# samanseifi/pyRMT

Hardware: AMD Instinct MI355X
Metric: cell-updates/s (full RMT step) at N=4096; achieved HBM GB/s vs peak (higher is better)
Workload: dtype f64; 1 GPU; soft_disc_in_lid_driven N=4096 semilagrangian (configs 2/4 loop body); grid=4096, parallelism=single-gpu

## Files before the change

include/rmt.h:

```cpp
#ifndef RMT_H
#define RMT_H

#ifdef __cplusplus
extern "C" {
#endif

typedef enum {
    RMT_OK = 0,
    RMT_EINVAL = 1,
    RMT_ENONFINITE = 2,
    RMT_EDEVICE = 3,
    RMT_ENOTSUP = 4,
    RMT_ENOMEM = 5
} rmt_status;

typedef enum {
    RMT_BC_NONE = 0,
    RMT_BC_NOSLIP_LID = 1,
    RMT_BC_FREESLIP_BOX = 2,
    RMT_BC_PERIODIC = 3
} rmt_bc_kind;

typedef enum {
    RMT_SCHEME_SEMILAGRANGIAN = 0,
// ... 54 lines not shown
int rmt_extrap_last_path(rmt_ctx *ctx, int *path);

int rmt_rebuild_phi_disc(rmt_ctx *ctx, const double *X1, const double *X2, double x0, double y0,
                         double R, double *phi);

int rmt_solid_cauchy_stress(rmt_ctx *ctx, const double *X1, const double *X2, double dx,
                            double dy, double mu_s, double kappa, const double *phi,
                            double w_cut, double detg_clamp, int isochoric, double *sxx,
                            double *sxy, double *syy, double *J);
int rmt_smoothed_heaviside(rmt_ctx *ctx, const double *x, long n, double w_t, double *H);
int rmt_apply_velocity_bc(rmt_ctx *ctx, int bc_kind, double lid, double *u, double *v);

typedef struct {
    int bc_kind;
    double lid;
    double mu_s, kappa, eta_s, rho_s, rho_f, mu_f, w_t;
    double dx, dy, dt;
    int stress_band;
    double detg_clamp;
} rmt_momentum_params;

int rmt_momentum_step_rk4(rmt_ctx *ctx, const rmt_momentum_params *prm, const double *u,
                          const double *v, const double *p, const double *X1, const double *X2,
                          const double *phi, double *u_new, double *v_new, double *sxx,
                          double *sxy, double *syy, double *J);
int rmt_compute_curvature(rmt_ctx *ctx, const double *phi, double dx, double dy, double *kappa);
int rmt_compute_contact_force(rmt_ctx *ctx, const double *phi1, const double *phi2, double k_rep,
                              double w_c, double dx, double dy, double *fx, double *fy);
int rmt_momentum_step_rk4_st(rmt_ctx *ctx, const rmt_momentum_params *prm, double gamma,
                             const double *u, const double *v, const double *p, const double *X1,
                             const double *X2, const double *phi, double *u_new, double *v_new,
                             double *sxx, double *sxy, double *syy, double *J);
int rmt_momentum_step_rk4_2solids(rmt_ctx *ctx, const rmt_momentum_params *prm, double k_rep,
                                  double w_c, const double *u, const double *v, const double *p,
                                  const double *X1a, const double *X2a, const double *X1b,
                                  const double *X2b, const double *phi_a, const double *phi_b,
                                  double *u_new, double *v_new, double *Jmin);

int rmt_mask_solid(rmt_ctx *ctx, const double *q, const double *phi, double *out);
int rmt_mixture_density(rmt_ctx *ctx, const double *phi_a, const double *phi_b, double w_t,
                        double rho_s, double rho_f, double *rho);
int rmt_two_solid_diag(rmt_ctx *ctx, const double *phi_a, const double *phi_b, const double *X,
                       const double *Y, const double *Jmin, double *out5);

int rmt_momentum_set_mode(int mode);

int rmt_divergence_rc(rmt_ctx *ctx, const double *a, const double *b, const double *p,
                      double d_f, double dx, double dy, double *divU);
int rmt_divergence_central(rmt_ctx *ctx, const double *a, const double *b, double dx,
                           double dy, double *divU);
int rmt_pressure_gradient(rmt_ctx *ctx, const double *p, double dx, double dy, double *gx,
                          double *gy);
int rmt_solve_poisson_dct(rmt_ctx *ctx, const double *rhs, double dx, double dy, double *p);
int rmt_pressure_projection(rmt_ctx *ctx, const double *a_star, const double *b_star,
                            double dx, double dy, double dt, double rho, int bc_kind,
                            double lid, const double *p_prev, double *a, double *b, double *p);
int rmt_pressure_projection_rho_field(rmt_ctx *ctx, const double *a_star, const double *b_star,
                                      double dx, double dy, double dt, const double *rho,
                                      int bc_kind, double lid, const double *p_prev, double *a,
                                      double *b, double *p);
int rmt_pressure_projection_variable(rmt_ctx *ctx, const double *a_star, const double *b_star,
                                     double dx, double dy, double dt, const double *rho,
                                     int bc_kind, double lid, const double *p_prev, double rtol,
                                     int maxiter, double *a, double *b, double *p, int *iters);
int rmt_apply_variable_poisson(rmt_ctx *ctx, const double *p, double dx, double dy,
                               const double *inv_rho, double *out);
int rmt_divergence_rc_variable(rmt_ctx *ctx, const double *a, const double *b, const double *p,
                               double dt, const double *rho, double dx, double dy,
                               double *divU);

int rmt_compute_timestep(rmt_ctx *ctx, const double *a, const double *b, double dx, double dy,
                         double CFL, double dt_min_cap, double mu_s, double rho_s, double gamma,
                         double rho_f, double mu_f, double eta_s, double kappa, double *dt);

int rmt_compute_kinetic_energy(rmt_ctx *ctx, const double *a, const double *b, double rho_f,
                               double rho_s, const double *phi, double w_t, double dx, double dy,
                               double *ke);
int rmt_compute_strain_energy(rmt_ctx *ctx, const double *X1, const double *X2, const double *phi,
                              double mu_s, double dx, double dy, double kappa, double *se);
int rmt_compute_viscous_dissipation(rmt_ctx *ctx, const double *a, const double *b, double mu_f,
                                    const double *phi, double w_t, double dx, double dy,
                                    double eta_s, double *diss);
int rmt_divergence_2d_interior(rmt_ctx *ctx, const double *u, const double *v, double dx,
                               double dy, int pad, double *div);
int rmt_velocity_rhs_blended(rmt_ctx *ctx, const double *u, const double *v, const double *p,
                             const double *sxx, const double *sxy, const double *syy, double dx,
                             double dy, double mu_f, const double *H, const double *rho,
                             const double *fx, const double *fy, double *rhs_u, double *rhs_v);

typedef enum {
    RMT_SHAPE_NONE = 0,
    RMT_SHAPE_DISC = 1
} rmt_shape_kind;

typedef struct {
    int ny, nx;
    double dx, dy;
    const double *xs, *ys;
    int scheme;
    int bc_kind;
    double lid;
    int shape;
    double x0, y0, R;
    double mu_s, kappa, rho_s, eta_s, mu_f, rho_f, w_t;
    int layers;
    double cfl, dt_cap;
// ... 142 lines not shown
```

pyrmt_amd/_lib.py:

```python
import ctypes
import os

_HERE = os.path.dirname(os.path.abspath(__file__))
LIB_PATH = os.environ.get("RMT_LIB") or os.path.join(_HERE, "librmt.so")

RMT_OK, RMT_EINVAL, RMT_ENONFINITE, RMT_EDEVICE, RMT_ENOTSUP, RMT_ENOMEM = range(6)


class RMTError(RuntimeError):
    pass


class rmt_momentum_params(ctypes.Structure):
    _fields_ = [("bc_kind", ctypes.c_int), ("lid", ctypes.c_double),
                ("mu_s", ctypes.c_double), ("kappa", ctypes.c_double),
                ("eta_s", ctypes.c_double), ("rho_s", ctypes.c_double),
                ("rho_f", ctypes.c_double), ("mu_f", ctypes.c_double), ("w_t", ctypes.c_double),
                ("dx", ctypes.c_double), ("dy", ctypes.c_double), ("dt", ctypes.c_double),
                ("stress_band", ctypes.c_int), ("detg_clamp", ctypes.c_double)]


class rmt_sim_params(ctypes.Structure):
    _fields_ = [("ny", ctypes.c_int), ("nx", ctypes.c_int),
                ("dx", ctypes.c_double), ("dy", ctypes.c_double),
# ... 30 lines not shown


_P, _D, _I, _L = ctypes.c_void_p, ctypes.c_double, ctypes.c_int, ctypes.c_long
SIGNATURES = {
    "rmt_last_error": (ctypes.c_char_p, []),
    "rmt_version": (_I, []),
    "rmt_ctx_create": (_I, [_I, _I, _I, _P, ctypes.POINTER(_P)]),
    "rmt_ctx_set_stream": (_I, [_P, _P]),
    "rmt_ctx_destroy": (_I, [_P]),
    "rmt_ctx_sync": (_I, [_P]),
    "rmt_ctx_set_profiling": (_I, [_P, _I]),
    "rmt_ctx_kernel_ms": (_I, [_P, ctypes.POINTER(_D)]),
    "rmt_ctx_set_option": (_I, [_P, ctypes.c_char_p, _I]),
    "rmt_ctx_get_option": (_I, [_P, ctypes.c_char_p, ctypes.POINTER(_I)]),
    "rmt_grad_x_2nd": (_I, [_P, _P, _D, _P]),
    "rmt_grad_y_2nd": (_I, [_P, _P, _D, _P]),
    "rmt_diff_upwind_3rd": (_I, [_P, _P, _P, _D, _I, _P]),
    "rmt_bilinear_interpolate": (_I, [_P, _P, _P, _P, _L, _D, _D, _P]),
    "rmt_advect_sl_rk4": (_I, [_P, _P, _P, _P, _P, _P, _D, _D, _D, _P]),
    "rmt_weno5_rhs": (_I, [_P, _P, _P, _P, _D, _D, _P, _D, _P]),
    "rmt_advect_weno5_rk3": (_I, [_P, _P, _P, _P, _D, _D, _D, _P, _D, _P]),
    "rmt_all_finite2": (_I, [_P, _P, _P, ctypes.POINTER(_I)]),
    "rmt_selftest_divk": (_I, [_P, _P, _L, _D, _P, _P]),
    "rmt_central_rhs": (_I, [_P, _P, _P, _P, _D, _D, _P, _D, _I, _P]),
    "rmt_advect_central_rk3": (_I, [_P, _P, _P, _P, _D, _D, _D, _P, _D, _I, _P]),
    "rmt_bicubic_interpolate": (_I, [_P, _P, _P, _P, _L, _D, _D, _P]),
    "rmt_advect_sl_cubic_rk4": (_I, [_P, _P, _P, _P, _P, _P, _D, _D, _D, _P]),
    "rmt_extrapolate_reference_map": (_I, [_P, _P, _P, _P, _D, _D, _I, _P, _P]),
    "rmt_extrap_set_mode": (_I, [_I]),
    "rmt_extrap_set_parallel": (_I, [_I]),
    "rmt_momentum_set_mode": (_I, [_I]),
    "rmt_extrap_last_path": (_I, [_P, ctypes.POINTER(_I)]),
    "rmt_rebuild_phi_disc": (_I, [_P, _P, _P, _D, _D, _D, _P]),
    "rmt_solid_cauchy_stress": (_I, [_P, _P, _P, _D, _D, _D, _D, _P, _D, _D, _I, _P, _P, _P, _P]),
    "rmt_smoothed_heaviside": (_I, [_P, _P, _L, _D, _P]),
    "rmt_apply_velocity_bc": (_I, [_P, _I, _D, _P, _P]),
    "rmt_momentum_step_rk4": (_I, [_P, ctypes.POINTER(rmt_momentum_params), _P, _P, _P, _P, _P,
                                   _P, _P, _P, _P, _P, _P, _P]),
    "rmt_compute_curvature": (_I, [_P, _P, _D, _D, _P]),
    "rmt_compute_contact_force": (_I, [_P, _P, _P, _D, _D, _D, _D, _P, _P]),
    "rmt_momentum_step_rk4_st": (_I, [_P, ctypes.POINTER(rmt_momentum_params), _D, _P, _P, _P,
                                      _P, _P, _P, _P, _P, _P, _P, _P, _P]),
    "rmt_momentum_step_rk4_2solids": (_I, [_P, ctypes.POINTER(rmt_momentum_params), _D, _D, _P,
                                           _P, _P, _P, _P, _P, _P, _P, _P, _P, _P, _P]),
    "rmt_mask_solid": (_I, [_P, _P, _P, _P]),
    "rmt_mixture_density": (_I, [_P, _P, _P, _D, _D, _D, _P]),
    "rmt_two_solid_diag": (_I, [_P, _P, _P, _P, _P, _P, ctypes.POINTER(_D)]),
    "rmt_pressure_projection_rho_field": (_I, [_P, _P, _P, _D, _D, _D, _P, _I, _D, _P, _P, _P,
                                               _P]),
    "rmt_divergence_rc": (_I, [_P, _P, _P, _P, _D, _D, _D, _P]),
    "rmt_divergence_central": (_I, [_P, _P, _P, _D, _D, _P]),
    "rmt_pressure_gradient": (_I, [_P, _P, _D, _D, _P, _P]),
    "rmt_solve_poisson_dct": (_I, [_P, _P, _D, _D, _P]),
    "rmt_pressure_projection": (_I, [_P, _P, _P, _D, _D, _D, _D, _I, _D, _P, _P, _P, _P]),
    "rmt_pressure_projection_variable": (_I, [_P, _P, _P, _D, _D, _D, _P, _I, _D, _P, _D, _I,
                                              _P, _P, _P, ctypes.POINTER(_I)]),
    "rmt_apply_variable_poisson": (_I, [_P, _P, _D, _D, _P, _P]),
    "rmt_divergence_rc_variable": (_I, [_P, _P, _P, _P, _D, _P, _D, _D, _P]),
    "rmt_compute_timestep": (_I, [_P, _P, _P, _D, _D, _D, _D, _D, _D, _D, _D, _D, _D, _D,
                                  ctypes.POINTER(_D)]),
    "rmt_divergence_2d_interior": (_I, [_P, _P, _P, _D, _D, _I, _P]),
    "rmt_compute_kinetic_energy": (_I, [_P, _P, _P, _D, _D, _P, _D, _D, _D, ctypes.POINTER(_D)]),
    "rmt_compute_strain_energy": (_I, [_P, _P, _P, _P, _D, _D, _D, _D, ctypes.POINTER(_D)]),
    "rmt_compute_viscous_dissipation": (_I, [_P, _P, _P, _D, _P, _D, _D, _D, _D,
                                             ctypes.POINTER(_D)]),
    "rmt_velocity_rhs_blended": (_I, [_P, _P, _P, _P, _P, _P, _P, _D, _D, _D, _P, _P, _P, _P,
                                      _P, _P]),
    "rmt_sim_create": (_I, [_P, ctypes.POINTER(rmt_sim_params), ctypes.POINTER(_P)]),
    "rmt_sim_destroy": (_I, [_P]),
    "rmt_sim_set_sync_every": (_I, [_P, _I]),
    "rmt_sim_field": (_I, [_P, _I, ctypes.POINTER(_P)]),
    "rmt_sim_step": (_I, [_P, _I, _D]),
    "rmt_sim_diagnostics": (_I, [_P, ctypes.POINTER(rmt_diag), _I, ctypes.POINTER(_I)]),
    "rmt_sim_set_profiling": (_I, [_P, _I]),
    "rmt_sim_set_carry": (_I, [_P, _I]),
    "rmt_sim_invalidate": (_I, [_P]),
    "rmt_sim_phase_times": (_I, [_P, ctypes.POINTER(_D), ctypes.POINTER(_L)]),
    "rmt_divergence_periodic": (_I, [_P, _P, _P, _D, _D, _P]),
    "rmt_pressure_gradient_periodic": (_I, [_P, _P, _D, _D, _P, _P]),
    "rmt_solve_poisson_fft": (_I, [_P, _P, _P, _P, _P]),
    "rmt_pressure_projection_periodic": (_I, [_P, _P, _P, _D, _D, _D, _D, _P, _I, _D, _P, _P,
                                              _P, _P, _P, _P]),
    "rmt_slab_create": (_I, [_P, ctypes.POINTER(rmt_sim_params), _I, _I, ctypes.POINTER(_I),
                             ctypes.POINTER(_I), ctypes.POINTER(_P)]),
    "rmt_slab_destroy": (_I, [_P]),
    "rmt_slab_info": (_I, [_P, ctypes.POINTER(_I), ctypes.POINTER(_D)]),
    "rmt_slab_buffer": (_I, [_P, _I, ctypes.POINTER(_P)]),
    "rmt_slab_begin": (_I, [_P]),
    "rmt_slab_advect_interior": (_I, [_P, _D]),
    "rmt_slab_advect": (_I, [_P, _D]),
    "rmt_slab_rim_pack": (_I, [_P]),
    "rmt_slab_extrapolate": (_I, [_P, _P, ctypes.POINTER(ctypes.c_longlong), ctypes.c_longlong]),
    "rmt_slab_momentum": (_I, [_P, _D]),
    "rmt_slab_project_rows": (_I, [_P, _D]),
    "rmt_slab_project_cols": (_I, [_P]),
    "rmt_slab_project_unrows": (_I, [_P]),
    "rmt_slab_sub_mean": (_I, [_P, _I, _P]),
    "rmt_slab_project_correct": (_I, [_P, _D]),
    "rmt_slab_finish": (_I, [_P]),
    "rmt_slab_set_device_dt": (_I, [_P, _I]),
    "rmt_slab_next_dt": (_I, [_P, _P, _I, _P]),
    "rmt_slab_rim_cap": (_I, [_P, ctypes.c_longlong]),
    "rmt_slab_next_bits": (_I, [_P]),
    "rmt_slab_geometry": (_I, [_P]),
    "rmt_slab_drop_geometry": (_I, [_P]),
    "rmt_slab_extrapolate_dev": (_I, [_P, _P, _P, ctypes.c_longlong]),
# ... 72 lines not shown
```

pyrmt_amd/csrc/ops.hip:

```cpp
#include "rmt_internal.hpp"
#include <algorithm>
#include <cstdio>
#include <cstring>
#include <mutex>
#include <vector>

namespace rmt {
static thread_local std::string g_err;
void set_error(const std::string &m) { g_err = m; }
static const struct { const char *name, *env; int rmt_opts::*f; } kOpts[] = {
    {"ext_events", "RMT_EXT_EVENTS", &rmt_opts::ext_events},
    {"ex_arena_bump", nullptr, &rmt_opts::ex_arena_bump},
    {"ex_profile", "RMT_EX_PROFILE", &rmt_opts::ex_profile},
    {"fix_all", "RMT_FIX_ALL", &rmt_opts::fix_all},
    {"dct_rocfft", "RMT_DCT_ROCFFT", &rmt_opts::dct_rocfft},
    {"transpose2", "RMT_TRANSPOSE2", &rmt_opts::transpose2},
    {"sim_hiprio", "RMT_SIM_HIPRIO", &rmt_opts::sim_hiprio},
    {"sim_sync", "RMT_SIM_SYNC", &rmt_opts::sim_sync},
    {"early_geometry", "RMT_EARLY_GEOMETRY", &rmt_opts::early_geometry},
    {"early_transpose", "RMT_EARLY_TRANSPOSE", &rmt_opts::early_transpose},
    {"fused_fluid", "RMT_FUSED_FLUID", &rmt_opts::fused_fluid},
    {"no_overlap", "RMT_NO_OVERLAP", &rmt_opts::no_overlap},
    {"side_tail", "RMT_SIDE_TAIL", &rmt_opts::side_tail},
    {"par_overlap", "RMT_PAR_OVERLAP", &rmt_opts::par_overlap},
    {"fused_fixprep", "RMT_FUSED_FIXPREP", &rmt_opts::fused_fixprep},
    {"merged_join", "RMT_MERGED_JOIN", &rmt_opts::merged_join},
    {"test_delay_side", "RMT_TEST_DELAY_SIDE", &rmt_opts::test_delay_side},
    {"test_delay_main", "RMT_TEST_DELAY_MAIN", &rmt_opts::test_delay_main},
    {"test_delay_geo", "RMT_TEST_DELAY_GEO", &rmt_opts::test_delay_geo},
    {"test_nowait_drop", "RMT_TEST_NOWAIT_DROP", &rmt_opts::test_nowait_drop},
    {"chain_cols", "RMT_CH_PARTS", &rmt_opts::ch_cols},
    {"chain_layer_groups", "RMT_CH_LAYERS", &rmt_opts::ch_lgroups},
    {"edge_slots", "RMT_EDGE_SLOTS_USED", &rmt_opts::edge_slots},
    {"edge_stream", "RMT_EDGE_STREAM", &rmt_opts::edge_stream},
    {"sl_phi", "RMT_SL_PHI", &rmt_opts::sl_phi},
    {"mac_boxes", "RMT_MAC_BOXES", &rmt_opts::mac_boxes},
    {"skip_marked_rows", "RMT_SKIP_MARKED_ROWS", &rmt_opts::skip_marked_rows},
    {"tail_stream", "RMT_TAIL_STREAM", &rmt_opts::tail_stream},
    {"diag_first", "RMT_DIAG_FIRST", &rmt_opts::diag_first},
    {"mac_noop_host", "RMT_MAC_NOOP_HOST", &rmt_opts::mac_noop_host},
    {"mac_face_sl", "RMT_MAC_FACE_SL", &rmt_opts::mac_face_sl},
    {"mac_m2_bound", "RMT_MAC_M2_BOUND", &rmt_opts::mac_m2_bound},
    {"diag_seg", "RMT_DIAG_SEG", &rmt_opts::diag_seg},
    {"sl_zero_flags", "RMT_SL_ZERO_FLAGS", &rmt_opts::sl_zero_flags},
    {"dct_desc", "RMT_DCT_DESC", &rmt_opts::dct_desc},
};
int g_list_blocks = getenv("RMT_LIST_BLOCKS") ? std::max(1, atoi(getenv("RMT_LIST_BLOCKS")))
                                                : LIST_BLOCKS;
static rmt_opts opts_from_env() {
    rmt_opts o;
    for (const auto &k : kOpts)
        if (k.env)
            if (const char *e = getenv(k.env)) o.*(k.f) = atoi(e);
    if (const char *e = getenv("RMT_EX_ARENA")) o.ex_arena_bump = !strcmp(e, "bump");
    o.test_delay_side = std::max(0, o.test_delay_side);
    o.test_delay_main = std::max(0, o.test_delay_main);
    o.test_delay_geo = std::max(0, o.test_delay_geo);
    return o;
}

int ensure_scratch(rmt_ctx *ctx, size_t bytes) {
    if (ctx->scratch_bytes >= bytes) return RMT_OK;
    RMT_HIP(hipDeviceSynchronize());
    if (ctx->scratch) RMT_HIP(hipFree(ctx->scratch));
    ctx->scratch = nullptr; ctx->scratch_bytes = 0;
    RMT_HIP(hipMalloc(&ctx->scratch, bytes));
    ctx->scratch_bytes = bytes;
    return RMT_OK;
}
int ensure_bytes(rmt_ctx *ctx, size_t bytes) {
    ++ctx->bytes_gen;
    if (ctx->bytes_len >= bytes) return RMT_OK;
    RMT_HIP(hipDeviceSynchronize());
    if (ctx->bytes) RMT_HIP(hipFree(ctx->bytes));
    ctx->bytes = nullptr; ctx->bytes_len = 0;
    RMT_HIP(hipMalloc(&ctx->bytes, bytes));
    ctx->bytes_len = bytes;
    return RMT_OK;
}


template <int OP>
__global__ void __launch_bounds__(RED_T) k_reduce_p1(const double *__restrict__ a,
                                                     const double *__restrict__ b, long n,
                                                     double *__restrict__ part) {
    __shared__ double s[RED_T];
    double acc = OP == 0 ? 0.0 : -INFINITY;
    for (long k = blockIdx.x * (long)RED_T + threadIdx.x; k < n; k += (long)RED_BLOCKS * RED_T) {
        double x = OP >= 2 ? a[k] * a[k] + b[k] * b[k] : a[k];
        if (OP == 0) acc += x;
        else if (OP == 3) acc = (x > acc || x != x) ? x : acc;
        else acc = fmax(acc, x);
    }
    s[threadIdx.x] = acc;
    __syncthreads();
    for (int w = RED_T / 2; w > 0; w >>= 1) {
        if (threadIdx.x < w)
            s[threadIdx.x] = OP == 0 ? s[threadIdx.x] + s[threadIdx.x + w]
// ... 829 lines not shown
    RMT_LAUNCHED();
    return RMT_OK;
}
int rmt_advect_sl_cubic_rk4(rmt_ctx *ctx, const double *q, const double *a, const double *b,
                            const double *X, const double *Y, double dt, double dx, double dy,
                            double *out) {
    k_sl_cubic<<<LAUNCH1D(N_CELLS)>>>(q, a, b, X, Y, ctx->ny, ctx->nx, dt, dx, dy, out);
    RMT_LAUNCHED();
    return RMT_OK;
}
int rmt_solid_cauchy_stress(rmt_ctx *ctx, const double *X1, const double *X2, double dx,
                            double dy, double mu_s, double kappa, const double *phi,
                            double w_cut, double detg_clamp, int isochoric, double *sxx,
                            double *sxy, double *syy, double *J) {
    k_solid_stress<<<LAUNCH1D(N_CELLS)>>>(X1, X2, phi, ctx->ny, ctx->nx, dx, dy, mu_s, kappa,
                                          w_cut, detg_clamp, isochoric, sxx, sxy, syy, J);
    RMT_LAUNCHED();
    return RMT_OK;
}
int rmt_smoothed_heaviside(rmt_ctx *ctx, const double *x, long n, double w_t, double *H) {
    if (n <= 0) return RMT_OK;
    k_heaviside<<<LAUNCH1D(n)>>>(x, n, w_t, H);
    RMT_LAUNCHED();
    return RMT_OK;
}
int rmt_apply_velocity_bc(rmt_ctx *ctx, int bc_kind, double lid, double *u, double *v) {
    RMT_CHECK(bc_kind >= 0 && bc_kind <= 3, RMT_EINVAL, "unknown velocity bc kind");
    k_apply_bc<<<LAUNCH1D(N_CELLS)>>>(bc_kind, lid, u, v, ctx->ny, ctx->nx);
    RMT_LAUNCHED();
    return RMT_OK;
}
int rmt_divergence_rc(rmt_ctx *ctx, const double *a, const double *b, const double *p,
                      double d_f, double dx, double dy, double *divU) {
    RMT_TRY(divergence_full(ctx->stream, a, b, p, ctx->ny, ctx->nx, d_f, rc_div(dx, dy), divU, 0.0,
                            1.0, nullptr));
    RMT_LAUNCHED();
    return RMT_OK;
}
int rmt_divergence_central(rmt_ctx *ctx, const double *a, const double *b, double dx,
                           double dy, double *divU) {
    k_divergence_central<<<LAUNCH1D(N_CELLS)>>>(a, b, ctx->ny, ctx->nx, dx, dy, divU);
    RMT_LAUNCHED();
    return RMT_OK;
}
int rmt_pressure_gradient(rmt_ctx *ctx, const double *p, double dx, double dy, double *gx,
                          double *gy) {
    k_pressure_gradient<<<LAUNCH1D(N_CELLS)>>>(p, ctx->ny, ctx->nx, dx, dy, gx, gy);
    RMT_LAUNCHED();
    return RMT_OK;
}
int rmt_solve_poisson_dct(rmt_ctx *ctx, const double *rhs, double dx, double dy, double *p) {
    return dct_solve(ctx, rhs, dx, dy, p);
}
int rmt_pressure_projection(rmt_ctx *ctx, const double *a_star, const double *b_star,
                            double dx, double dy, double dt, double rho, int bc_kind,
                            double lid, const double *p_prev, double *a, double *b, double *p) {
    RMT_CHECK(bc_kind >= 0 && bc_kind <= 3, RMT_EINVAL, "unknown velocity bc kind");
    long n = N_CELLS;
    RMT_TRY(ensure_scratch(ctx, 2 * n * sizeof(double)));
    double *rhs = ctx->scratch, *pc = rhs + n;
    if (p_prev && rho > 0) {
        RMT_TRY(divergence_full(ctx->stream, a_star, b_star, p_prev, ctx->ny, ctx->nx, dt / rho,
                                rc_div(dx, dy), rhs, rho, dt, nullptr));
        RMT_LAUNCHED();
    } else {
        if (p_prev) RMT_TRY(rmt_divergence_rc(ctx, a_star, b_star, p_prev, dt / rho, dx, dy, rhs));
        else RMT_TRY(rmt_divergence_central(ctx, a_star, b_star, dx, dy, rhs));
        k_scale_copy<<<LAUNCH1D(n)>>>(rhs, n, rho, rhs);
        k_div_scalar<<<LAUNCH1D(n)>>>(rhs, n, dt, rhs);
    }
    double *root = ctx->red + RED_BLOCKS + 17;
    RMT_TRY(dct_solve(ctx, rhs, dx, dy, pc, root));
    k_project_correct<<<rows_grid(ctx->nx, 0, ctx->ny), 256, 0, ctx->stream>>>(a_star, b_star, pc, p_prev, ctx->ny, ctx->nx, divk_make(2 * dx), divk_make(2 * dy),
                                       dt / rho, bc_kind, lid, a, b, p, 0, ctx->ny, root, (double)n);
    RMT_LAUNCHED();
    RMT_TRY(sub_mean_rows(ctx, p, ctx->ny, ctx->nx));
    return RMT_OK;
}
int rmt_compute_timestep(rmt_ctx *ctx, const double *a, const double *b, double dx, double dy,
                         double CFL, double dt_min_cap, double mu_s, double rho_s, double gamma,
                         double rho_f, double mu_f, double eta_s, double kappa, double *dt) {
    (void)dy;
    RMT_TRY(reduce_maxsq2(ctx, a, b, N_CELLS, ctx->red + RED_BLOCKS));
    double m2;
    RMT_TRY(read_scalar(ctx, ctx->red + RED_BLOCKS, &m2));
    double cs = std::sqrt((kappa + mu_s * 4.0 / 3.0) / (rho_s + 1e-12));
    double d = CFL * dx / (cs + 1e-14);
    d = std::fmin(d, CFL * dx / (std::sqrt(m2) + 1e-6));
    if (gamma > 1e-12) {
        double ra = 0.5 * (rho_s + rho_f);
        d = std::fmin(d, std::sqrt((ra * std::pow(dx, 3.0)) / (2 * M_PI * gamma)) * 0.5);
    } else {
        d = std::fmin(d, 1.0);
    }
    double mu_max = std::fmax(mu_f, eta_s), rho_min = std::fmin(rho_s, rho_f);
    d = std::fmin(d, (mu_max > 1e-12 && rho_min > 1e-12) ? CFL * rho_min * std::pow(dx, 2.0) / (4.0 * mu_max)
                                                         : 1.0);
    *dt = std::fmin(d, dt_min_cap);
    return RMT_OK;
}
}

namespace rmt {
int projection_rows(rmt_ctx *ctx, const double *a_star, const double *b_star, double dx,
                    double dy, const double *dtp, double dt, double rho, const double *p_prev,
                    const unsigned char *rowmark, const int *tiles, const int *tcount,
// ... 59 lines not shown
```

pyrmt_amd/csrc/poisson.hip:

```cpp
#include "rmt_internal.hpp"
#include "dft_consts.hpp"
#include <algorithm>
#include <vector>

namespace rmt {

struct DctPlan {
    int ny = 0, nx = 0;
    rocfft_plan px = nullptr, py = nullptr;
    rocfft_execution_info info = nullptr;
    void *work = nullptr;
    size_t work_bytes = 0;
    double *E = nullptr;
    double *C = nullptr;
    double *T = nullptr;
    double *lamx = nullptr, *lamy = nullptr;
    double dx = 0, dy = 0;
    bool lds = false;
    int big = 0;
    int mat = 0;
    double2 *Wx = nullptr, *Wy = nullptr;
    int radx[16] = {0}, rady[16] = {0}, npx = 0, npy = 0;
};

static bool g_rocfft_ready = false;

static int rf(rocfft_status s, const char *what) {
    if (s != rocfft_status_success) {
        set_error(std::string("rocFFT: ") + what + " failed (" + std::to_string((int)s) + ")");
        return RMT_EDEVICE;
    }
    return RMT_OK;
}

static int make_r2c(rocfft_plan *plan, size_t M, size_t batch) {
    rocfft_plan_description d = nullptr;
    RMT_TRY(rf(rocfft_plan_description_create(&d), "description_create"));
    size_t istr = 1, ostr = 1, idist = M, odist = M / 2 + 1;
    RMT_TRY(rf(rocfft_plan_description_set_data_layout(d, rocfft_array_type_real,
                                                       rocfft_array_type_hermitian_interleaved,
                                                       nullptr, nullptr, 1, &istr, idist, 1, &ostr,
                                                       odist), "set_data_layout"));
    int s = rf(rocfft_plan_create(plan, rocfft_placement_notinplace,
                                  rocfft_transform_type_real_forward, rocfft_precision_double, 1,
                                  &M, batch, d), "plan_create");
    rocfft_plan_description_destroy(d);
    return s;
}

void dct_destroy(DctPlan *P) {
    if (!P) return;
    if (P->px) rocfft_plan_destroy(P->px);
    if (P->py) rocfft_plan_destroy(P->py);
    if (P->info) rocfft_execution_info_destroy(P->info);
    (void)hipFree(P->work); (void)hipFree(P->E); (void)hipFree(P->C); (void)hipFree(P->T);
    (void)hipFree(P->lamx); (void)hipFree(P->lamy);
    (void)hipFree(P->Wx); (void)hipFree(P->Wy);
    delete P;
}

static void host_lambda(int n, double h, std::vector<double> &lam) {
    lam.resize(n);
    double h2 = std::pow(h, 2.0);
    for (int k = 0; k < n; ++k) lam[k] = -2.0 * (1.0 - std::cos(M_PI * k / (n - 1))) / h2;
}

constexpr int DCT_MAXM = 8192;
constexpr int K1_MAXN = DCT_MAXM / 2;

static bool is_mat_radix(int R) { return R == 29 || R == 31; }
static bool factor(int M, int *rad, int *np, bool mat = false, bool desc = false) {
    if (M < 2 || M > DCT_MAXM) return false;
    int cnt[32] = {0}, m = M;
    for (int q : {2, 3, 5, 7, 11, 13, 17, 19, 23})
        while (m % q == 0) { ++cnt[q]; m /= q; }
    if (mat)
        for (int q : {29, 31})
            while (m % q == 0) { ++cnt[q]; m /= q; }
    if (m != 1) return false;
    int n = 0;
    auto put = [&](int r) { if (n < 16) rad[n++] = r; };
    while (cnt[2] >= 3) { put(8); cnt[2] -= 3; }
    if (cnt[2] == 2) { put(4); cnt[2] = 0; }
    while (cnt[3] >= 2) { put(9); cnt[3] -= 2; }
    if (cnt[2] && cnt[5]) { put(10); --cnt[2]; --cnt[5]; }
    if (cnt[2] && cnt[3]) { put(6); --cnt[2]; --cnt[3]; }
    for (int q : {2, 3, 5, 7, 11, 13, 17, 19, 23, 29, 31})
        while (cnt[q]) { put(q); --cnt[q]; }
    std::sort(rad, rad + n);
    if (desc) std::reverse(rad, rad + n);
    *np = n;
    return n < 16;
}

static bool big_radix(const int *rad, int np) {
    for (int k = 0; k < np; ++k) if (rad[k] > 13 && !is_mat_radix(rad[k])) return true;
    return false;
}
static bool mat_radix(const int *rad, int np) {
    for (int k = 0; k < np; ++k) if (is_mat_radix(rad[k])) return true;
    return false;
}

static double2 unit_root(long t, long L) {
    const long double PI = 3.141592653589793238462643383279502884L;
    t %= L;
    if ((4 * t) % L == 0) {
        const int e = (int)(4 * t / L);
        const double c[4] = {1.0, 0.0, -1.0, 0.0}, sn[4] = {0.0, 1.0, 0.0, -1.0};
        return make_double2(c[e], -sn[e]);
    }
    const long double a = 2.0L * PI * t / L;
    return make_double2((double)cosl(a), (double)-sinl(a));
}
static int twiddles(int M, const int *rad, int np, double2 **W, bool post = false) {
    std::vector<double2> h;
    h.reserve(2 * (size_t)M + 2);
    int Ns = 1;
    for (int q = 0; q < np; ++q) {
        const int R = rad[q], L = Ns * R;
        for (int r = 1; r < R; ++r)
            for (int k = 0; k < Ns; ++k) h.push_back(unit_root((long)k * r, L));
        Ns = L;
    }
    if (post)
        for (long k = 0; k <= M; ++k) h.push_back(unit_root(k, 2L * M));
    h.push_back(make_double2(1.0, 0.0));
    RMT_HIP(hipMalloc(W, h.size() * sizeof(double2)));
    RMT_UPLOAD(*W, h.data(), h.size() * sizeof(double2));
    return RMT_OK;
}

constexpr size_t FFT_LDS_MAX = 160 * 1024 - 4096;
static bool lds_fits(int M) { return (size_t)M * sizeof(double2) <= FFT_LDS_MAX; }

int dct_plan(rmt_ctx *ctx, double dx, double dy) {
    DctPlan *P = ctx->dct;
    if (P && P->dx == dx && P->dy == dy) return RMT_OK;
    if (!P) {
        P = ctx->dct = new DctPlan;
        P->ny = ctx->ny; P->nx = ctx->nx;
        const int Nx = P->nx - 1, Ny = P->ny - 1;
        P->lds = !ctx->opt.dct_rocfft && Nx >= 2 && Ny >= 2 && Nx < K1_MAXN && Ny < K1_MAXN &&
                 factor(Nx, P->radx, &P->npx, true, ctx->opt.dct_desc && Nx == 4095) &&
                 factor(Ny, P->rady, &P->npy, true, ctx->opt.dct_desc && Ny == 4095) &&
                 lds_fits(Nx) && lds_fits(Ny);
        P->big = big_radix(P->radx, P->npx) || big_radix(P->rady, P->npy);
        P->mat = mat_radix(P->radx, P->npx) || mat_radix(P->rady, P->npy);
        if (P->mat) P->lds = P->lds && lds_fits(2 * Nx + 64) && lds_fits(2 * Ny + 64);
    }
    if (!P->lds && !g_rocfft_ready) { RMT_TRY(rf(rocfft_setup(), "setup")); g_rocfft_ready = true; }
    if (P->lds && !P->Wx) {
        const size_t n = (size_t)P->ny * P->nx;
        RMT_TRY(twiddles(P->nx - 1, P->radx, P->npx, &P->Wx, true));
        RMT_TRY(twiddles(P->ny - 1, P->rady, P->npy, &P->Wy, true));
        RMT_HIP(hipMalloc(&P->T, n * sizeof(double)));
        RMT_HIP(hipMalloc(&P->lamx, P->nx * sizeof(double)));
        RMT_HIP(hipMalloc(&P->lamy, P->ny * sizeof(double)));
    }
    if (!P->lds && !P->px) {
        size_t Mx = 2 * (size_t)(P->nx - 1), My = 2 * (size_t)(P->ny - 1);
        RMT_TRY(make_r2c(&P->px, Mx, P->ny));
        if (P->ny == P->nx) P->py = nullptr;
        else RMT_TRY(make_r2c(&P->py, My, P->nx));
        size_t w1 = 0, w2 = 0;
        rocfft_plan_get_work_buffer_size(P->px, &w1);
        if (P->py) rocfft_plan_get_work_buffer_size(P->py, &w2);
        P->work_bytes = std::max(w1, w2);
        if (P->work_bytes) RMT_HIP(hipMalloc(&P->work, P->work_bytes));
        RMT_TRY(rf(rocfft_execution_info_create(&P->info), "execution_info_create"));
        if (P->work_bytes)
            RMT_TRY(rf(rocfft_execution_info_set_work_buffer(P->info, P->work, P->work_bytes),
                       "set_work_buffer"));
        size_t ne = std::max((size_t)P->ny * Mx, (size_t)P->nx * My);
        size_t n = (size_t)P->ny * P->nx;
        RMT_HIP(hipMalloc(&P->E, ne * sizeof(double)));
        RMT_HIP(hipMalloc(&P->C, 2 * n * sizeof(double)));
        RMT_HIP(hipMalloc(&P->T, n * sizeof(double)));
        RMT_HIP(hipMalloc(&P->lamx, P->nx * sizeof(double)));
        RMT_HIP(hipMalloc(&P->lamy, P->ny * sizeof(double)));
    }
    std::vector<double> lx, ly;
    host_lambda(P->nx, dx, lx);
    host_lambda(P->ny, dy, ly);
    RMT_UPLOAD(P->lamx, lx.data(), lx.size() * 8);
    RMT_UPLOAD(P->lamy, ly.data(), ly.size() * 8);
    P->dx = dx; P->dy = dy;
    return RMT_OK;
}

__global__ void k_even_ext(const double *__restrict__ src, int rows, int n,
                           double *__restrict__ E) {
    const long M = 2L * (n - 1);
    long q = blockIdx.x * (long)blockDim.x + threadIdx.x;
    if (q >= (long)rows * M) return;
    long r = q / M, k = q % M;
    E[q] = src[r * n + (k < n ? k : M - k)];
}

constexpr int TT = 32;
__global__ void __launch_bounds__(TT * 8) k_real_T(const double *__restrict__ C, int rows, int n,
                                                   double scale, const double *__restrict__ lamr,
                                                   const double *__restrict__ lamk,
                                                   double *__restrict__ out) {
    __shared__ double tile[TT][TT + 1];
    int k0 = blockIdx.x * TT, r0 = blockIdx.y * TT;
    for (int rr = threadIdx.y; rr < TT; rr += 8) {
        int r = r0 + rr, k = k0 + threadIdx.x;
// ... 353 lines not shown
            const int kx = row0 + r;
            __syncthreads();
#pragma unroll
            for (int t = 0; t < PP; ++t) {
                const int k = tid + t * NT;
                if (k <= N / 2) {
                    const double ea = (kx == 0 && k == 0) ? 1.0 : lr[kx] + lk[k];
                    const double ya = xa[t] / ea;
                    d[k] = ya;
                    if (k >= 1) d[2 * N - k] = ya;
                    const int kb = N - k;
                    if (kb != k) {
                        const double yb = xb[t] / (lr[kx] + lk[kb]);
                        d[kb] = yb;
                        if (kb >= 1 && kb < N) d[2 * N - kb] = yb;
                    }
                }
                __builtin_amdgcn_sched_barrier(0);
            }
            continue;
        }
        double *o = dst + (long)r * n;
#pragma unroll
        for (int t = 0; t < PP; ++t) {
            const int k = tid + t * NT;
            if (k <= N / 2) {
                o[k] = xa[t] * scale;
                if (N - k != k) o[N - k] = xb[t] * scale;
            }
        }
        if (rs) {
            __syncthreads();
#pragma unroll
            for (int t = 0; t < PP; ++t) {
                const int k = tid + t * NT;
                if (k <= N / 2) { d[k] = xa[t] * scale; d[N - k] = xb[t] * scale; }
            }
            __syncthreads();
            if (tid < 256) {
                double acc = 0.0;
                for (int k = tid; k < n; k += 256) acc += d[k];
                red[tid] = acc;
            }
            __syncthreads();
            for (int w = 128; w > 0; w >>= 1) {
                if (tid < w) red[tid] = red[tid] + red[tid + w];
                __syncthreads();
            }
            if (tid == 0) rs[r] = red[0];
        }
    }
}

__global__ void __launch_bounds__(256) k_transpose(const double *__restrict__ in, int R, int C,
                                                   double *__restrict__ out,
                                                   const unsigned char *__restrict__ rowmark = nullptr,
                                                   int mode = 0) {
    __shared__ double t[64][65];
    const int c0 = blockIdx.x * 64, r0 = blockIdx.y * 64, tx = threadIdx.x & 63, ty = threadIdx.x >> 6;
    if (rowmark) {
        const bool any = __syncthreads_or(threadIdx.x < 64 && r0 + tx < R && rowmark[r0 + tx] != 0);
        if (any != (mode == 2)) return;
    }
    for (int rr = ty; rr < 64; rr += 4) {
        const int r = r0 + rr, c = c0 + tx;
        if (r < R && c < C) t[rr][tx] = in[(long)r * C + c];
    }
    __syncthreads();
    for (int cc = ty; cc < 64; cc += 4) {
        const int c = c0 + cc, r = r0 + tx;
        if (r < R && c < C) out[(long)c * R + r] = t[tx][cc];
    }
}

static Radices radices(const int *rad, int np) {
    Radices rd{};
    int Ns = 1, off = 0;
    for (int k = 0; k < np; ++k) {
        rd.p[k] = Pass{rad[k], Ns, (float)(1.0 / Ns), off};
        off += (rad[k] - 1) * Ns;
        Ns *= rad[k];
    }
    rd.n = np;
    return rd;
}

int dct_pass(rmt_ctx *ctx, bool solve, int axis, const double *src, double *dst, int nrows,
             int row0, double scale, double *rs, const unsigned char *rowmark, bool unmarked) {
    DctPlan *P = ctx->dct;
    RMT_CHECK(P && P->lds, RMT_ENOTSUP, "dct_pass: no LDS DCT plan for this grid");
    RMT_CHECK(!solve || axis == 1, RMT_EINVAL, "dct_pass: the solve pass runs along y");
    RMT_CHECK(!rs || (!solve && nrows <= ctx->rsum_len), RMT_EINVAL, "dct_pass: row sums");
    RMT_CHECK(!rowmark || (!solve && !rs), RMT_EINVAL, "dct_pass: row marks on a plain row pass");
    static bool attr = false;
    if (!attr) {
        const void *fs[8] = {(const void *)k_dct1<false, 0>, (const void *)k_dct1<true, 0>,
                             (const void *)k_dct1<false, 1>, (const void *)k_dct1<true, 1>,
                             (const void *)k_dct1<false, 0, 1>, (const void *)k_dct1<true, 0, 1>,
                             (const void *)k_dct1<false, 0, 3>, (const void *)k_dct1<true, 0, 3>};
        for (auto f : fs)
            RMT_HIP(hipFuncSetAttribute(f, hipFuncAttributeMaxDynamicSharedMemorySize,
                                        (int)FFT_LDS_MAX));
        attr = true;
    }
    if (nrows <= 0) return RMT_OK;
    const int n = axis == 0 ? P->nx : P->ny;
    const int *rad = axis == 0 ? P->radx : P->rady, np = axis == 0 ? P->npx : P->npy;
    const Radices rd = radices(rad, np);
    const double2 *W = axis == 0 ? P->Wx : P->Wy;
    const size_t lds = (size_t)(P->mat ? 2 * (n - 1) + 32 : n - 1) * sizeof(double2);
    const unsigned g = (unsigned)nrows;
    hipStream_t st = ctx->stream;
    const bool k4095 = n == 4096 && !P->big && np == 4 && rad[0] == 5 &&
                       rad[1] == 7 && rad[2] == 9 && rad[3] == 13;
    const bool k4095d = n == 4096 && !P->big && np == 4 && rad[0] == 13 &&
                        rad[1] == 9 && rad[2] == 7 && rad[3] == 5;
    if (k4095d && solve)
        k_dct1<true, 0, 3><<<g, K1T<0>::T, lds, st>>>(src, dst, nrows, n, W, rd, scale, P->lamx, P->lamy, row0, nullptr, nullptr);
    else if (k4095d)
        k_dct1<false, 0, 3><<<g, K1T<0>::T, lds, st>>>(src, dst, nrows, n, W, rd, scale, nullptr, nullptr, 0, rs, rowmark, unmarked);
    else if (k4095 && solve)
        k_dct1<true, 0, 1><<<g, K1T<0>::T, lds, st>>>(src, dst, nrows, n, W, rd, scale, P->lamx, P->lamy, row0, nullptr, nullptr);
    else if (k4095)
        k_dct1<false, 0, 1><<<g, K1T<0>::T, lds, st>>>(src, dst, nrows, n, W, rd, scale, nullptr, nullptr, 0, rs, rowmark, unmarked);
    else if (solve) {
        if (P->big) k_dct1<true, 1><<<g, K1T<1>::T, lds, st>>>(src, dst, nrows, n, W, rd, scale, P->lamx, P->lamy, row0, nullptr, nullptr);
        else k_dct1<true, 0><<<g, K1T<0>::T, lds, st>>>(src, dst, nrows, n, W, rd, scale, P->lamx, P->lamy, row0, nullptr, nullptr);
    } else {
        if (P->big) k_dct1<false, 1><<<g, K1T<1>::T, lds, st>>>(src, dst, nrows, n, W, rd, scale, nullptr, nullptr, 0, rs, rowmark, unmarked);
        else k_dct1<false, 0><<<g, K1T<0>::T, lds, st>>>(src, dst, nrows, n, W, rd, scale, nullptr, nullptr, 0, rs, rowmark, unmarked);
    }
    RMT_LAUNCHED();
    return RMT_OK;
}

bool dct_lds_ready(rmt_ctx *ctx) { return ctx->dct && ctx->dct->lds; }

__global__ void __launch_bounds__(256) k_transpose2(const double *__restrict__ in, int R, int C,
                                                    double *__restrict__ out,
                                                    const unsigned char *__restrict__ rowmark,
                                                    int mode) {
    __shared__ double t[64][65];
    const int c0 = blockIdx.x * 64, r0 = blockIdx.y * 64, tx = threadIdx.x & 31, ty = threadIdx.x >> 5;
    if (rowmark) {
        const int l = threadIdx.x & 63;
        const bool any = __syncthreads_or(threadIdx.x < 64 && r0 + l < R && rowmark[r0 + l] != 0);
        if (any != (mode == 2)) return;
    }
    double2 v[8];
#pragma unroll
    for (int k = 0; k < 8; ++k) {
        const int r = r0 + ty + 8 * k, c = c0 + 2 * tx;
        v[k] = (r < R && c < C) ? *(const double2 *)(in + (long)r * C + c) : make_double2(0.0, 0.0);
    }
#pragma unroll
    for (int k = 0; k < 8; ++k) {
        t[ty + 8 * k][2 * tx] = v[k].x;
        t[ty + 8 * k][2 * tx + 1] = v[k].y;
    }
    __syncthreads();
#pragma unroll
    for (int k = 0; k < 8; ++k) {
        const int c = c0 + ty + 8 * k, r = r0 + 2 * tx;
        if (c < C && r < R)
            *(double2 *)(out + (long)c * R + r) = make_double2(t[2 * tx][ty + 8 * k], t[2 * tx + 1][ty + 8 * k]);
// ... 291 lines not shown
```

pyrmt_amd/csrc/rmt_internal.hpp:

```cpp
#pragma once
#include <hip/hip_runtime.h>
#include <hip/hip_ext.h>
#include <rocfft/rocfft.h>
#include <algorithm>
#include <cmath>
#include <cstdint>
#include <string>
#include "../../include/rmt.h"
#include "divk.hpp"

namespace rmt {

constexpr int LIST_BLOCKS = 1024;
extern int g_list_blocks;
inline unsigned list_grid(long max_tiles) {
    return (unsigned)std::max(1L, std::min<long>(max_tiles, g_list_blocks));
}

__host__ __device__ __forceinline__ double nanmax(double a, double b) {
    return (a != a || b != b) ? (a + b) : (a > b ? a : b);
}


void set_error(const std::string &msg);
// ... 17 lines not shown
#define RMT_CHECK(cond, code, msg)                                                      \
    do {                                                                                \
        if (!(cond)) { ::rmt::set_error(msg); return (code); }                          \
    } while (0)
#define RMT_UPLOAD(dst, src, bytes)                                                     \
    do {                                                                                \
        RMT_HIP(hipMemcpy((dst), (src), (bytes), hipMemcpyHostToDevice));               \
        RMT_HIP(hipDeviceSynchronize());                                                \
    } while (0)
#define RMT_TRY(expr)                                                                   \
    do { int s_ = (expr); if (s_ != RMT_OK) return s_; } while (0)

struct DctPlan;
struct Dct2Plan;
struct PerPlan;

}

struct rmt_opts {
    int ext_events = 1;
    int ex_arena_bump = 0;
    int ex_profile = 0;
    int fix_all = 0;
    int dct_rocfft = 0;
    int transpose2 = 1;
    int sim_hiprio = 1;
    int sim_sync = 0;
    int early_geometry = 1;
    int early_transpose = 1;
    int fused_fluid = 1;
    int no_overlap = 0;
    int side_tail = 1;
    int par_overlap = 1;
    int fused_fixprep = 1;
    int merged_join = 1;
    int test_delay_side = 0;
    int test_delay_main = 0;
    int test_delay_geo = 0;
    int test_nowait_drop = 0;
    int ch_cols = 2;
    int ch_lgroups = 0;
    int edge_slots = 64;
    int edge_stream = 1;
    int sl_phi = 1;
    int mac_boxes = 1;
    int skip_marked_rows = 1;
    int tail_stream = 1;
    int diag_first = 0;
    int mac_noop_host = 1;
    int mac_face_sl = 1;
    int mac_m2_bound = 1;
    int diag_seg = 1;
    int dct_desc = 1;
    int sl_zero_flags = 1;
};

#define RMT_EDGE_PRIOS 2
#ifndef RMT_EDGE_SLOTS
#define RMT_EDGE_SLOTS 64
#endif
struct rmt_ctx {
    int ny = 0, nx = 0, device = 0;
    hipStream_t stream = nullptr;
    double *scratch = nullptr;
    size_t scratch_bytes = 0;
    double *red = nullptr;
    double *rsum = nullptr;
    int rsum_len = 0;
    unsigned char *bytes = nullptr;
    size_t bytes_len = 0;
    unsigned long bytes_gen = 0;
    rmt::DctPlan *dct = nullptr;
    rmt::Dct2Plan *dct2 = nullptr;
    rmt::PerPlan *per = nullptr;
    bool prof = false;
    hipEvent_t ev[4] = {nullptr, nullptr, nullptr, nullptr};
    int ex_layers = 0;
    bool ex_chain = false;
    bool ex_par = false;
    bool ex_noop_skip = false;
    struct EdgeTiles { int *list = nullptr; int n = 0; long key[6] = {}; };
    EdgeTiles edge[RMT_EDGE_SLOTS];
    int edge_next = 0;
    hipStream_t edge_sts[RMT_EDGE_PRIOS] = {};
    int edge_prios[RMT_EDGE_PRIOS] = {};
    hipEvent_t edge_ev[9] = {};
    void *imex[2] = {nullptr, nullptr};
    rmt_opts opt;
};
static_assert(sizeof(((rmt_ctx *)nullptr)->edge) / sizeof(rmt_ctx::EdgeTiles) == RMT_EDGE_SLOTS, "edge slots");

namespace rmt {

struct StreamScope {
    rmt_ctx *ctx;
    hipStream_t prev;
    StreamScope(rmt_ctx *c, hipStream_t s) : ctx(c), prev(c->stream) { c->stream = s; }
    ~StreamScope() { ctx->stream = prev; }
    StreamScope(const StreamScope &) = delete;
    StreamScope &operator=(const StreamScope &) = delete;
};

int ensure_scratch(rmt_ctx *ctx, size_t bytes);
int ensure_bytes(rmt_ctx *ctx, size_t bytes);
inline unsigned grid1d(long n, int block) { return (unsigned)((n + block - 1) / block); }

// ... 532 lines not shown
```

Before: 5.562 billion cell-updates/s.

## Add symmetry-exploiting half-length DCT kernel for Poisson row transforms

Adds a new DCT-I row kernel that uses the even symmetry of the extended sequence. It stores only half the complex data in LDS, uses prime-factor radix passes over symmetric index pairs, and reads the output through a precomputed index table. This roughly halves LDS footprint and butterfly work per row compared with the existing full-length k_dct1 path, and is enabled by default through a new dct_sym option. The cost is a more complex indexing scheme, a new table upload, and a self-test entry point to validate row sums.

```diff
diff --git a/include/rmt.h b/include/rmt.h
--- a/include/rmt.h
+++ b/include/rmt.h
@@ -130,6 +130,9 @@
 int rmt_pressure_gradient(rmt_ctx *ctx, const double *p, double dx, double dy, double *gx,
                           double *gy);
 int rmt_solve_poisson_dct(rmt_ctx *ctx, const double *rhs, double dx, double dy, double *p);
+int rmt_selftest_dct_rows(rmt_ctx *ctx, const double *src, double dx, double dy, double scale,
+                          double *dst, double *rs, double *rs_ref,
+                          const unsigned char *rowmark, int unmarked);
 int rmt_pressure_projection(rmt_ctx *ctx, const double *a_star, const double *b_star,
                             double dx, double dy, double dt, double rho, int bc_kind,
                             double lid, const double *p_prev, double *a, double *b, double *p);
diff --git a/pyrmt_amd/_lib.py b/pyrmt_amd/_lib.py
--- a/pyrmt_amd/_lib.py
+++ b/pyrmt_amd/_lib.py
@@ -106,6 +106,7 @@
     "rmt_divergence_central": (_I, [_P, _P, _P, _D, _D, _P]),
     "rmt_pressure_gradient": (_I, [_P, _P, _D, _D, _P, _P]),
     "rmt_solve_poisson_dct": (_I, [_P, _P, _D, _D, _P]),
+    "rmt_selftest_dct_rows": (_I, [_P, _P, _D, _D, _D, _P, _P, _P, _P, _I]),
     "rmt_pressure_projection": (_I, [_P, _P, _P, _D, _D, _D, _D, _I, _D, _P, _P, _P, _P]),
     "rmt_pressure_projection_variable": (_I, [_P, _P, _P, _D, _D, _D, _P, _I, _D, _P, _D, _I,
                                               _P, _P, _P, ctypes.POINTER(_I)]),
diff --git a/pyrmt_amd/csrc/ops.hip b/pyrmt_amd/csrc/ops.hip
--- a/pyrmt_amd/csrc/ops.hip
+++ b/pyrmt_amd/csrc/ops.hip
@@ -44,6 +44,7 @@
     {"diag_seg", "RMT_DIAG_SEG", &rmt_opts::diag_seg},
     {"sl_zero_flags", "RMT_SL_ZERO_FLAGS", &rmt_opts::sl_zero_flags},
     {"dct_desc", "RMT_DCT_DESC", &rmt_opts::dct_desc},
+    {"dct_sym", "RMT_DCT_SYM", &rmt_opts::dct_sym},
 };
 int g_list_blocks = getenv("RMT_LIST_BLOCKS") ? std::max(1, atoi(getenv("RMT_LIST_BLOCKS")))
                                                 : LIST_BLOCKS;
@@ -979,6 +980,18 @@
 int rmt_solve_poisson_dct(rmt_ctx *ctx, const double *rhs, double dx, double dy, double *p) {
     return dct_solve(ctx, rhs, dx, dy, p);
 }
+int rmt_selftest_dct_rows(rmt_ctx *ctx, const double *src, double dx, double dy, double scale,
+                          double *dst, double *rs, double *rs_ref,
+                          const unsigned char *rowmark, int unmarked) {
+    RMT_CHECK(ctx && src && dst, RMT_EINVAL, "null argument");
+    RMT_TRY(dct_plan(ctx, dx, dy));
+    RMT_TRY(dct_pass(ctx, false, 0, src, dst, ctx->ny, 0, scale, rs, rowmark, unmarked != 0));
+    if (rs_ref) {
+        k_rowsum<<<ctx->ny, 256, 0, ctx->stream>>>(dst, ctx->nx, rs_ref);
+        RMT_LAUNCHED();
+    }
+    return RMT_OK;
+}
 int rmt_pressure_projection(rmt_ctx *ctx, const double *a_star, const double *b_star,
                             double dx, double dy, double dt, double rho, int bc_kind,
                             double lid, const double *p_prev, double *a, double *b, double *p) {
diff --git a/pyrmt_amd/csrc/poisson.hip b/pyrmt_amd/csrc/poisson.hip
--- a/pyrmt_amd/csrc/poisson.hip
+++ b/pyrmt_amd/csrc/poisson.hip
@@ -21,6 +21,8 @@
     int mat = 0;
     double2 *Wx = nullptr, *Wy = nullptr;
     int radx[16] = {0}, rady[16] = {0}, npx = 0, npy = 0;
+    int symx[4] = {0}, symy[4] = {0}, nsx = 0, nsy = 0;
+    unsigned short *tabx = nullptr, *taby = nullptr;
 };
 
 static bool g_rocfft_ready = false;
@@ -56,6 +58,7 @@
     (void)hipFree(P->work); (void)hipFree(P->E); (void)hipFree(P->C); (void)hipFree(P->T);
     (void)hipFree(P->lamx); (void)hipFree(P->lamy);
     (void)hipFree(P->Wx); (void)hipFree(P->Wy);
+    (void)hipFree(P->tabx); (void)hipFree(P->taby);
     delete P;
 }
 
@@ -131,6 +134,27 @@
     return RMT_OK;
 }
 
+static bool sym_factor(int N, int *rad, int *np) {
+    int n = 0, m = N;
+    for (int R : {13, 11, 9, 7, 5, 3})
+        if (m % R == 0 && n < 4 && !(R == 3 && N % 9 == 0)) { rad[n++] = R; m /= R; }
+    *np = n;
+    return N >= 3 && N < K1_MAXN && m == 1;
+}
+static int sym_table(int N, const int *rad, int np, unsigned short **tab) {
+    std::vector<unsigned short> h((N + 1) / 2);
+    for (int k = 0; k <= (N - 1) / 2; ++k) {
+        const long k2 = (long)k * ((N + 1) / 2) % N;
+        long sig = 0;
+        for (int q = 0; q < np; ++q) sig += (k2 % rad[q]) * (N / rad[q]);
+        sig %= N;
+        h[k] = (unsigned short)std::min(sig, N - sig);
+    }
+    RMT_HIP(hipMalloc(tab, h.size() * sizeof(unsigned short)));
+    RMT_UPLOAD(*tab, h.data(), h.size() * sizeof(unsigned short));
+    return RMT_OK;
+}
+
 constexpr size_t FFT_LDS_MAX = 160 * 1024 - 4096;
 static bool lds_fits(int M) { return (size_t)M * sizeof(double2) <= FFT_LDS_MAX; }
 
@@ -148,12 +172,16 @@
         P->big = big_radix(P->radx, P->npx) || big_radix(P->rady, P->npy);
         P->mat = mat_radix(P->radx, P->npx) || mat_radix(P->rady, P->npy);
         if (P->mat) P->lds = P->lds && lds_fits(2 * Nx + 64) && lds_fits(2 * Ny + 64);
+        if (!(P->lds && ctx->opt.dct_sym && sym_factor(Nx, P->symx, &P->nsx))) P->nsx = 0;
+        if (!(P->lds && ctx->opt.dct_sym && sym_factor(Ny, P->symy, &P->nsy))) P->nsy = 0;
     }
     if (!P->lds && !g_rocfft_ready) { RMT_TRY(rf(rocfft_setup(), "setup")); g_rocfft_ready = true; }
     if (P->lds && !P->Wx) {
         const size_t n = (size_t)P->ny * P->nx;
         RMT_TRY(twiddles(P->nx - 1, P->radx, P->npx, &P->Wx, true));
         RMT_TRY(twiddles(P->ny - 1, P->rady, P->npy, &P->Wy, true));
+        if (P->nsx) RMT_TRY(sym_table(P->nx - 1, P->symx, P->nsx, &P->tabx));
+        if (P->nsy) RMT_TRY(sym_table(P->ny - 1, P->symy, P->nsy, &P->taby));
         RMT_HIP(hipMalloc(&P->T, n * sizeof(double)));
         RMT_HIP(hipMalloc(&P->lamx, P->nx * sizeof(double)));
         RMT_HIP(hipMalloc(&P->lamy, P->ny * sizeof(double)));
@@ -613,6 +641,170 @@
     }
 }
 
+constexpr int K1S_T = 256;
+struct SymRad { int R[4]; int n; };
+
+template <int R, int NT, int NMAX>
+__device__ __forceinline__ void sym_pass(double2 *z, const int N, const int s) {
+    constexpr int LPT = ((NMAX / R + 1) / 2 + NT - 1) / NT;
+    const int nl = (s + 1) / 2;
+    int tid = threadIdx.x;
+    asm volatile("" : "+v"(tid));
+    double2 v[LPT][R];
+#pragma unroll
+    for (int b = 0; b < LPT; ++b) {
+        const int q = tid + b * NT;
+        if (q < nl) {
+#pragma unroll
+            for (int j = 0; j < R; ++j) {
+                int i = R * q + j * s;
+                if (i >= N) i -= N;
+                v[b][j] = z[min(i, N - i)];
+            }
+        }
+    }
+    __syncthreads();
+    asm volatile("" : "+v"(tid));
+#pragma unroll
+    for (int b = 0; b < LPT; ++b) {
+        const int q = tid + b * NT;
+        if (q < nl) {
+            dft<R>(v[b]);
+#pragma unroll
+            for (int k = 0; k < R; ++k) {
+                int i = R * q + k * s;
+                if (i >= N) i -= N;
+                if (k <= R / 2 || q != 0) z[min(i, N - i)] = v[b][k];
+            }
+        }
+    }
+    __syncthreads();
+}
+
+template <bool SOLVE, bool K4095>
+__global__ void __launch_bounds__(K1S_T, 4) k_dct1s(const double *__restrict__ src,
+                                                    double *__restrict__ dst, int rows, int n,
+                                                    const unsigned short *__restrict__ tab,
+                                                    SymRad sr, double scale,
+                                                    const double *__restrict__ lamr,
+                                                    const double *__restrict__ lamk, int row0,
+                                                    double *__restrict__ rs,
+                                                    const unsigned char *__restrict__ rowmark,
+                                                    int rm_inv = 0) {
+    if (rowmark && (rowmark[blockIdx.x] != 0) == (rm_inv != 0)) return;
+    constexpr int NT = K1S_T;
+    constexpr int PP = (K1_MAXN / 2 + NT - 1) / NT;
+    extern __shared__ double2 z[];
+    __shared__ double red[256];
+    const int N = K4095 ? 4095 : n - 1, H = N / 2, r = blockIdx.x;
+    double *d = (double *)z;
+    {
+        const double *x = src + (long)r * n;
+        double va[PP], vb[PP];
+#pragma unroll
+        for (int t = 0; t < PP; ++t) {
+            const int m = threadIdx.x + t * NT;
+            if (K4095 || m <= H) { va[t] = x[m]; vb[t] = x[N - m]; }
+        }
+#pragma unroll
+        for (int t = 0; t < PP; ++t) {
+            const int m = threadIdx.x + t * NT;
+            if (K4095 || m <= H) z[m] = (m & 1) ? make_double2(vb[t], va[t]) : make_double2(va[t], vb[t]);
+        }
+    }
+#pragma unroll 1
+    for (int it = 0; it < (SOLVE ? 2 : 1); ++it) {
+        __syncthreads();
+        if constexpr (K4095) {
+            sym_pass<13, NT, 4095>(z, 4095, 315);
+            sym_pass<9, NT, 4095>(z, 4095, 455);
+            sym_pass<7, NT, 4095>(z, 4095, 585);
+            sym_pass<5, NT, 4095>(z, 4095, 819);
+        } else {
+            for (int q = 0; q < sr.n; ++q) {
+                const int s = N / sr.R[q];
+                switch (sr.R[q]) {
+                    case 3: sym_pass<3, NT, K1_MAXN>(z, N, s); break;
+                    case 5: sym_pass<5, NT, K1_MAXN>(z, N, s); break;
+                    case 7: sym_pass<7, NT, K1_MAXN>(z, N, s); break;
+                    case 9: sym_pass<9, NT, K1_MAXN>(z, N, s); break;
+                    case 11: sym_pass<11, NT, K1_MAXN>(z, N, s); break;
+                    case 13: sym_pass<13, NT, K1_MAXN>(z, N, s); break;
+                }
+            }
+        }
+        const unsigned short *tb = tab;
+        const double *lr = lamr, *lk = lamk;
+        int tid = threadIdx.x;
+        asm volatile("" : "+v"(tid));
+        int sl[PP];
+#pragma unroll
+        for (int t = 0; t < PP; ++t) {
+            const int k = tid + t * NT;
+            if (K4095 || k <= H) sl[t] = tb[k];
+        }
+        double xa[PP], xb[PP];
+#pragma unroll
+        for (int t = 0; t < PP; ++t) {
+            const int k = tid + t * NT;
+            if (K4095 || k <= H) {
+                const double2 C = z[sl[t]];
+                const double im = (k & 1) ? -C.y : C.y;
+                xa[t] = C.x + im;
+                xb[t] = C.x - im;
+            } else {
+                xa[t] = xb[t] = 0.0;
+            }
+        }
+        if (SOLVE && it == 0) {
+            const int kx = row0 + r;
+            const double lx = lr[kx];
+#pragma unroll
+            for (int t = 0; t < PP; ++t) {
+                const int k = tid + t * NT;
+                if (K4095 || k <= H) {
+                    const double ea = (kx == 0 && k == 0) ? 1.0 : lx + lk[k];
+                    xa[t] = xa[t] / ea;
+                    xb[t] = xb[t] / (lx + lk[N - k]);
+                }
+                __builtin_amdgcn_sched_barrier(0);
+            }
+            __syncthreads();
+#pragma unroll
+            for (int t = 0; t < PP; ++t) {
+                const int k = tid + t * NT;
+                if (K4095 || k <= H) z[k] = (k & 1) ? make_double2(xb[t], xa[t]) : make_double2(xa[t], xb[t]);
+            }
+            continue;
+        }
+        double *o = dst + (long)r * n;
+#pragma unroll
+        for (int t = 0; t < PP; ++t) {
+            const int k = tid + t * NT;
+            if (K4095 || k <= H) { o[k] = xa[t] * scale; o[N - k] = xb[t] * scale; }
+        }
+        if (rs) {
+            __syncthreads();
+#pragma unroll
+            for (int t = 0; t < PP; ++t) {
+                const int k = tid + t * NT;
+                if (K4095 || k <= H) { d[k] = xa[t] * scale; d[N - k] = xb[t] * scale; }
+            }
+            __syncthreads();
+            double acc = 0.0;
+            for (int k = tid; k < n; k += 256) acc += d[k];
+            red[tid] = acc;
+            __syncthreads();
+            for (int w = 128; w > 0; w >>= 1) {
+                if (tid < w) red[tid] = red[tid] + red[tid + w];
+                __syncthreads();
+            }
+            if (tid == 0) rs[r] = red[0];
+        }
+    }
+}
+static_assert(K1S_T == 256, "k_dct1s: the row sum is k_rowsum's, 256 partials");
+
 __global__ void __launch_bounds__(256) k_transpose(const double *__restrict__ in, int R, int C,
                                                    double *__restrict__ out,
                                                    const unsigned char *__restrict__ rowmark = nullptr,
@@ -672,6 +864,25 @@
     const size_t lds = (size_t)(P->mat ? 2 * (n - 1) + 32 : n - 1) * sizeof(double2);
     const unsigned g = (unsigned)nrows;
     hipStream_t st = ctx->stream;
+    if (const int ns = axis == 0 ? P->nsx : P->nsy) {
+        const int *sym = axis == 0 ? P->symx : P->symy;
+        const unsigned short *tab = axis == 0 ? P->tabx : P->taby;
+        SymRad sr{};
+        for (int k = 0; k < ns; ++k) sr.R[k] = sym[k];
+        sr.n = ns;
+        const size_t ldh = (size_t)n * sizeof(double);
+        const bool k4095 = n == 4096;
+        if (solve && k4095)
+            k_dct1s<true, true><<<g, K1S_T, ldh, st>>>(src, dst, nrows, n, tab, sr, scale, P->lamx, P->lamy, row0, nullptr, nullptr);
+        else if (solve)
+            k_dct1s<true, false><<<g, K1S_T, ldh, st>>>(src, dst, nrows, n, tab, sr, scale, P->lamx, P->lamy, row0, nullptr, nullptr);
+        else if (k4095)
+            k_dct1s<false, true><<<g, K1S_T, ldh, st>>>(src, dst, nrows, n, tab, sr, scale, nullptr, nullptr, 0, rs, rowmark, unmarked);
+        else
+            k_dct1s<false, false><<<g, K1S_T, ldh, st>>>(src, dst, nrows, n, tab, sr, scale, nullptr, nullptr, 0, rs, rowmark, unmarked);
+        RMT_LAUNCHED();
+        return RMT_OK;
+    }
     const bool k4095 = n == 4096 && !P->big && np == 4 && rad[0] == 5 &&
                        rad[1] == 7 && rad[2] == 9 && rad[3] == 13;
     const bool k4095d = n == 4096 && !P->big && np == 4 && rad[0] == 13 &&
diff --git a/pyrmt_amd/csrc/rmt_internal.hpp b/pyrmt_amd/csrc/rmt_internal.hpp
--- a/pyrmt_amd/csrc/rmt_internal.hpp
+++ b/pyrmt_amd/csrc/rmt_internal.hpp
@@ -93,6 +93,7 @@
     int mac_m2_bound = 1;
     int diag_seg = 1;
     int dct_desc = 1;
+    int dct_sym = 1;
     int sl_zero_flags = 1;
 };
 
```

Measured after the change: 5.663 billion cell-updates/s, median of 6. 1.02x the previous value.
